# anatshafir1/bpp-phyl

Hardware: AMD Instinct MI355X
Metric: site-pattern x node partial updates/s (higher is better)
Workload: dtype f64

## Files before the change

bpp-phyl_amd/csrc/plk.hip:

```cpp

#include "../../include/plk.h"
#include "plk_kernels.hpp"
#include "plk_tree4.hpp"
#include "plk_deriv.hpp"
#include "plk_mfma64.hpp"
#include "plk_treeM.hpp"
#include "plk_jit.hpp"
#include "plk_jitm.hpp"
#include "plk_dr.hpp"
#include "plk_post.hpp"
#include "plk_map.hpp"
#include "plk_nni.hpp"
#include "plk_rell.hpp"
#include "plk_pair.hpp"
#include "plk_pars.hpp"
#include "plk_sim.hpp"
#include "plk_smap.hpp"
#include "plk_exchange.hpp"

#include <hip/hip_runtime.h>
#include <hip/hiprtc.h>
#include <rccl/rccl.h>

#include <sys/stat.h>
// ... 280 lines not shown
  double* d_cls = nullptr;
  size_t d_cls_cap = 0;
  double* fused_cls_blocks = nullptr;
  bool cls_site_written = false;
  uint8_t* d_ucodes_dc = nullptr;
  size_t ucodes_dc_cap = 0;
  bool ucodes_dc_valid = false;
  int ucodes_dc_w = 0;
  int32_t* d_units_start = nullptr;
  size_t units_start_cap = 0;
  uint8_t* d_ucodes = nullptr;
  int4* d_units = nullptr;
  size_t ucodes_cap = 0, units_cap = 0;
  bool ucodes_valid = false;
  int jit_resident = 0;
  std::string kernel_path;
  std::vector<std::vector<uint8_t> > tip_codes_host;
  bool cmp_valid = false;
  bool slots_expanded = false;
  std::vector<plk_op> cmp_ops;
  std::vector<std::vector<int32_t> > cmp_ids;
  std::vector<int64_t> cmp_D;
  std::vector<int> cmp_level_start, cmp_level_maxD;
  uint32_t* d_links = nullptr;
  size_t d_links_cap = 0;
  KOpL* d_opsl = nullptr;
  KKid* d_kidsl = nullptr;
  size_t d_kidsl_cap = 0;
  size_t d_opsl_cap = 0;
  int64_t cmp_work = 0;
// ... 226 lines not shown
int collect_events(plk_handle h) {
  if (h->events.empty()) return PLK_OK;
  HIPCHK(h, hipStreamSynchronize(h->stream));
  for (auto& e : h->events) {
    float ms = 0.f;
    HIPCHK(h, hipEventElapsedTime(&ms, e.a, e.b));
    h->acc_ms[e.kind] += ms;
    h->event_pool.push_back(e);
  }
  h->events.clear();
  return PLK_OK;
}

std::mutex g_jit_mutex;
std::map<std::pair<int, std::string>, hipFunction_t> g_jit_cache;
std::map<std::string, std::vector<char> > g_jit_code;

std::string jit_cache_dir() {
  const char* e = env_get("PLK_JIT_CACHE");
  if (e && (e[0] == '0' || e[0] == '\0')) return std::string();
  std::string d;
  if (e) {
    d = e;
  } else if (const char* x = env_get("XDG_CACHE_HOME")) {
    d = std::string(x) + "/plk_jit";
  } else if (const char* hm = env_get("HOME")) {
    d = std::string(hm) + "/.cache/plk_jit";
  } else {
    return std::string();
  }
// ... 85 lines not shown
  hiprtcDestroyProgram(&prog);
  if (log)
    std::fprintf(stderr, "[plk] jit compiled %zu bytes of source in %.2f s\n", src.size(),
                 std::chrono::duration<double>(std::chrono::steady_clock::now() - t0).count());
  if (!stem.empty()) {
    write_file_atomic(stem + ".co", code->data(), code->size());
    const std::string sm = code_sum(*code);
    write_file_atomic(stem + ".sum", sm.data(), sm.size());
    write_file_atomic(stem + ".hip", src.data(), src.size());
  }
  return PLK_OK;
}

int jit_function(plk_handle h, const std::string& src, const char* name, hipFunction_t* out) {
  std::lock_guard<std::mutex> lock(g_jit_mutex);
  const auto key = std::make_pair(h->device, src);
  auto it = g_jit_cache.find(key);
  if (it != g_jit_cache.end()) {
    *out = it->second;
    return PLK_OK;
  }
  auto ct = g_jit_code.find(src);
  bool from_cache = false;
  if (ct == g_jit_code.end()) {
    std::vector<char> code;
    if (int rc = jit_compile(h, src, &code, false, &from_cache)) return rc;
    ct = g_jit_code.emplace(src, std::move(code)).first;
  }
  std::vector<char>& code = ct->second;
  if (const char* dir = env_get("PLK_JIT_DUMP")) {
    const std::string stem = std::string(dir) + "/plk_jit_" + std::to_string(g_jit_cache.size());
    if (FILE* f = std::fopen((stem + ".hip").c_str(), "wb")) {
      std::fwrite(src.data(), 1, src.size(), f);
      std::fclose(f);
// ... 6 lines not shown
  hipSetDevice(h->device);
  hipModule_t mod;
  auto load = [&]() {
    try {
      return hipModuleLoadData(&mod, code.data()) == hipSuccess;
    } catch (...) {
      return false;
    }
  };
  if (!load()) {
    if (!from_cache) return fail(h, PLK_ERR_DEVICE, "hipModuleLoadData of the compiled tree kernel failed");
    (void)hipGetLastError();
    if (int rc = jit_compile(h, src, &code, true, &from_cache)) return rc;
    if (!load()) return fail(h, PLK_ERR_DEVICE, "hipModuleLoadData of the recompiled tree kernel failed");
  }
  hipFunction_t fn;
  HIPCHK(h, hipModuleGetFunction(&fn, mod, name));
  g_jit_cache.emplace(key, fn);
  *out = fn;
  return PLK_OK;
}

bool s4_supported(int C) { return C == 1 || C == 2 || C == 4 || C == 8; }

constexpr int kDerivScratch = 6;
constexpr int kScratchMats = 4;
constexpr int kScratchTips = 4;

template <bool SCALE>
void launch_s4(plk_handle h, const KOp* d_ops, int n_ops, const PartialsArgs& a) {
// ... 79 lines not shown
    return PLK_OK;
  if (!h->table_set) return fail(h, PLK_ERR_STATE, "code table not set (plk_set_code_table)");
  for (int t = 0; t < h->n_tips; ++t)
    if (!h->pmat_valid[t]) return fail(h, PLK_ERR_STATE, "transition matrix of tip branch %d not set", t);
  if (h->n_tips > 0) {
    dim3 grid(h->n_tips, h->C);
    if (h->S == 64)
      tip_table64_kernel<<<grid, 256, (size_t)(64 * 64 + h->n_codes * 64) * sizeof(double), h->stream>>>(
          h->pmats, h->code_table, h->tipP, h->n_tips, h->C, h->n_codes);
    else
      tip_table_kernel<<<grid, 256, 0, h->stream>>>(h->pmats, h->code_table, h->tipP, h->n_tips, h->C, h->S,
                                                    h->n_codes);
    HIPCHK(h, hipGetLastError());
  }
  std::fill(h->tip_table_valid.begin(), h->tip_table_valid.end(), 1);
  return PLK_OK;
}

int upload_compact_table(plk_handle h) {
  const int S = h->S;
  const int U = std::max((int)h->code_orig.size(), 1);
  std::vector<double> t((size_t)U * S, 0.0);
  for (size_t k = 0; k < h->code_orig.size(); ++k)
    std::copy(h->code_table_host.begin() + (size_t)h->code_orig[k] * S,
              h->code_table_host.begin() + (size_t)(h->code_orig[k] + 1) * S, t.begin() + k * S);
  hipSetDevice(h->device);
  HIPCHK(h, hipStreamSynchronize(h->stream));
  HIPCHK(h, hipMemcpy(h->code_table, t.data(), t.size() * sizeof(double), hipMemcpyHostToDevice));
  h->n_codes = U;
  h->tip_table_valid.assign(h->n_tips, 0);
  return PLK_OK;
}

int multi_forward(plk_handle h, int rc) {
  if (rc) {
    h->last_error = std::string("shard: ") + g_last_error;
    for (plk_handle s : h->shards)
      if (!s->last_error.empty()) h->last_error = "shard: " + s->last_error;
  }
  return rc;
}

int multi_run(plk_handle h, const std::function<int(size_t)>& f) {
  const size_t n = h->shards.size();
  if (n == 1) {
// ... 15 lines not shown

int multi_slices(plk_handle h, const std::function<int(plk_handle, int64_t)>& f) {
  return multi_run(h, [&](size_t i) { return f(h->shards[i], h->shard_start[i]); });
}

}

extern "C" {
int root_launch_c(plk_handle h, int root, double* site_lnl);
int root_finish_c(plk_handle h, double* lnl, double* block_sums);
}

namespace {
double* block_target(plk_handle h);
int launch_cls_blocks(plk_handle h, int guard, int32_t* uflow, bool site);

int32_t* uflow_arm(plk_handle h) {
  if (h->flags & PLK_FLAG_SCALING) return nullptr;
  *(volatile int32_t*)h->h_uflow = 0;
  return h->d_uflow;
}

size_t shard_block0(plk_handle h, size_t i) { return (size_t)(h->shard_start[i] / kRootBlock); }

void sum_blocks(const std::vector<double>& all, double* lnl, double* block_sums) {
  double s = 0.0;
  for (double v : all) s += v;
  if (lnl) *lnl = s;
  if (block_sums) std::memcpy(block_sums, all.data(), all.size() * sizeof(double));
}
// ... 226 lines not shown
    delete h;
    return PLK_OK;
  }
  hipSetDevice(h->device);
  if (h->stream) hipStreamSynchronize(h->stream);
  comm_release(h);
  void* bufs[] = {h->partials, h->scale, h->codes, h->code_table, h->tipP, h->pmats, h->dpmats, h->d2pmats,
                  h->V, h->Vinv, h->lambda, h->weights, h->rates, h->probs, h->pi, h->site_lnl,
                  h->d_ops, h->wave_sums, h->d_links, h->d_opsl, h->d_prog, h->d_frag, h->d1_sums,
                  h->d2_sums, h->d_dprog, h->pmatsT, h->d_ucodes, h->d_units, h->d_cherry3,
                  h->d_cherry_tips, h->d_cherry, h->d_drb, h->d_drm, h->dr_blk, h->dr_out, h->d_drpre, h->d_sbctr,
                  h->d_cherry_rows, h->d_kidsl, h->d_cls, h->d_ucodes_dc, h->d_units_start, h->d_post, h->post_buf,
                  h->count_G, h->wmats, h->d_mapb, h->map_blk, h->d_mapreq, h->d_nni, h->nni_vit, h->d_pair,
                  h->rell_rows, h->rell_W, h->rell_stage, h->rell_bad, h->pars_sets, h->pars_scores, h->d_pars,
                  h->d_pars_moves, h->sim_states, h->d_sim, h->d_smap_tab, h->d_smap_pois, h->d_smap_list,
                  h->d_smap_sums, h->d_smap_work, h->d_smap_keep};
  for (void* p : bufs)
    if (p) hipFree(p);
  if (h->h_req) (void)hipHostFree(h->h_req);
  if (h->h_blocks) hipHostFree(h->h_blocks);
  if (h->h_uflow) hipHostFree(h->h_uflow);
  if (h->h_clk) hipHostFree(h->h_clk);
  if (h->h_nni) (void)hipHostFree(h->h_nni);
  if (h->req_done) hipEventDestroy(h->req_done);
  for (auto& e : h->events) {
    hipEventDestroy(e.a);
    hipEventDestroy(e.b);
  }
  for (auto& e : h->event_pool) {
    hipEventDestroy(e.a);
    hipEventDestroy(e.b);
// ... 293 lines not shown
  a.mask = deriv_mask;
  a.n_req = n;
  a.uni_model = -1;
  if (h->S == 64) {
    a.uni_model = model ? model[0] : 0;
    for (int i = 1; model && i < n; ++i)
      if (model[i] != a.uni_model) a.uni_model = -1;
  }
  const bool k64 = h->S == 64 && deriv_mask == PLK_DERIV_P;
  const bool tips_fused = h->table_set && (h->S <= 20 || (k64 && h->n_codes <= 64));
  a.init = tips_fused ? h->code_table : nullptr;
  a.tipP = h->tipP;
  a.n_tips = h->n_tips;
  a.n_codes = h->n_codes;
  TimedSpan span(h, PLK_TIME_PMAT, 1);
  const size_t lds = (size_t)(h->S + (tips_fused ? 3 : 2) * S2) * sizeof(double);
  const bool pk_generic = !k64 && h->S != 4;
  if ((k64 || pk_generic) && (deriv_mask & PLK_DERIV_P)) a.PT = h->pmatsT;
  if (k64) {
    const int rx = tune_int("P64RX", 4, 0, 4), nb = tune_int("P64NB", 2, 1, 4);
    if (rx == 0) {
      pmat64s_kernel<<<dim3(n, h->C, 4), dim3(256), (size_t)(64 + 16 * 64 + S2) * sizeof(double), h->stream>>>(a, inl);
    } else {
      const int rr = rx <= 1 ? 1 : rx <= 2 ? 2 : 4, nn = nb <= 1 ? 1 : nb <= 2 ? 2 : 4;
      const dim3 g((unsigned)((n * h->C + nn - 1) / nn), (unsigned)(64 / (4 * rr)));
      const size_t lds = (size_t)(64 * kP64Pad + nn * 64 + nn * 4 * rr * kP64Pad) * sizeof(double);
#define PLK_P64W(RX_, NB_) \
  if (rr == RX_ && nn == NB_) pmat64w_kernel<RX_, NB_><<<g, dim3(256), lds, h->stream>>>(a, inl);
      PLK_P64W(1, 1) PLK_P64W(1, 2) PLK_P64W(1, 4) PLK_P64W(2, 1) PLK_P64W(2, 2) PLK_P64W(2, 4)
      PLK_P64W(4, 1) PLK_P64W(4, 2) PLK_P64W(4, 4)
#undef PLK_P64W
    }
  } else if (h->S == 4)
  {
    const dim3 g4((unsigned)((n * h->C * 4 + 63) / 64));
    if (inl.n > 0 && inl.n <= kPmatInlineSmall) {
      PmatInlineSmall sm;
      sm.n = inl.n;
      std::copy(inl.t, inl.t + inl.n, sm.t);
      std::copy(inl.branch, inl.branch + inl.n, sm.branch);
      std::copy(inl.model, inl.model + inl.n, sm.model);
      pmat4_kernel<PmatInlineSmall><<<g4, dim3(64), 0, h->stream>>>(a, sm);
    } else {
      pmat4_kernel<PmatInline><<<g4, dim3(64), 0, h->stream>>>(a, inl);
    }
  }
  else
// ... 8 lines not shown
  }
  HIPCHK(h, hipGetLastError());
  if (inl.n == 0) {
    if (h->in_eval)
      h->req_unrecorded = true;
    else
      HIPCHK(h, hipEventRecord(h->req_done, h->stream));
  }
  span.stop();
  if (deriv_mask & PLK_DERIV_P) {
    for (int i = 0; i < n; ++i) {
      h->pmat_valid[branch[i]] = 1;
      if (!a.PT) h->pmatsT_dirty = true;
      if (branch[i] < h->n_tips) h->tip_table_valid[branch[i]] = tips_fused ? 1 : 0;
    }
  }
  if (h->deriv_valid.empty()) h->deriv_valid.assign(h->n_nodes, 0);
  const bool both = (deriv_mask & (PLK_DERIV_P | PLK_DERIV_DP | PLK_DERIV_D2P)) ==
                    (PLK_DERIV_P | PLK_DERIV_DP | PLK_DERIV_D2P);
  for (int i = 0; i < n; ++i) h->deriv_valid[branch[i]] = both ? 1 : 0;
  return PLK_OK;
}

int plk_set_pmatrix(plk_handle h, int branch, const double* P) {
  env_refresh();
  if (h && !h->shards.empty()) return multi_each(h, [&](plk_handle x) { return plk_set_pmatrix(x, branch, P); });
  if (!h || !P || branch < 0 || branch >= h->n_nodes) return fail(h, PLK_ERR_ARG, "bad branch %d", branch);
  hipSetDevice(h->device);
  HIPCHK(h, hipStreamSynchronize(h->stream));
  const size_t n = (size_t)h->C * h->S * h->S;
  HIPCHK(h, hipMemcpy(h->pmats + (size_t)branch * n, P, n * sizeof(double), hipMemcpyHostToDevice));
  h->pmat_valid[branch] = 1;
  h->state_epoch++;
  h->pmatsT_dirty = true;
  if (!h->deriv_valid.empty()) h->deriv_valid[branch] = 0;
  if (branch < h->n_tips) h->tip_table_valid[branch] = 0;
  return PLK_OK;
}

int plk_get_dpmatrix(plk_handle h, int branch, int order, double* dP) {
  env_refresh();
  if (h && !h->shards.empty()) return multi_forward(h, plk_get_dpmatrix(h->shards[0], branch, order, dP));
  if (!h || !dP || branch < 0 || branch >= h->n_nodes || (order != 1 && order != 2))
    return fail(h, PLK_ERR_ARG, "bad derivative request (branch %d, order %d)", branch, order);
  const double* src = order == 1 ? h->dpmats : h->d2pmats;
  if (!src) return fail(h, PLK_ERR_STATE, "no derivative matrices (PLK_DERIV_DP / PLK_DERIV_D2P)");
  hipSetDevice(h->device);
  HIPCHK(h, hipStreamSynchronize(h->stream));
  const size_t n = (size_t)h->C * h->S * h->S;
  HIPCHK(h, hipMemcpy(dP, src + (size_t)branch * n, n * sizeof(double), hipMemcpyDeviceToHost));
  return PLK_OK;
// ... 298 lines not shown
  for (int i = 0; i < nf; ++i) {
    start_sorted[i] = start[order[i]];
    start_sorted[nf + i] = res_first[order[i]];
    if (h->prog_tiers.empty() || tier[order[i]] != tier[order[i - 1]]) h->prog_tiers.push_back({});
    h->prog_tiers.back().push_back(i);
  }
  HIPCHK(h, hipMemcpyAsync(h->d_frag, start_sorted.data(), 2 * nf * sizeof(int32_t), hipMemcpyHostToDevice,
                           h->stream));
  h->prog_nf = nf;
  rc = ensure_cap(h, (void**)&h->d_sbctr, &h->d_sbctr_cap, (size_t)(nf * h->C + 1) * sizeof(unsigned));
  if (rc) return rc;
  HIPCHK(h, hipMemsetAsync(h->d_sbctr, 0, (size_t)(nf * h->C + 1) * sizeof(unsigned), h->stream));
  h->prog_host = prog;
  h->frag_starts_host.assign(start_sorted.begin(), start_sorted.begin() + nf);
  h->jit_fn = nullptr;
  h->jitm_fn = nullptr;
  h->jit_plan_valid = false;
  HIPCHK(h, hipStreamSynchronize(h->stream));
  h->prog_ops.assign(ops, ops + n_ops);
  h->prog_materialize = materialize;
  h->prog_reduce = reduce;
  h->prog_dm = DM;
  h->prog_jit = jit_tree4(h);
  h->prog_jitm = jit_treeM(h);
  h->prog_ciw = jit_ciw(h);
  h->prog_tmax = TMAX;
  h->prog_root = root_reduce;
  h->cherry3.swap(cherry3);
  h->cherry_codes_valid = false;
  h->prog_mat_after.assign(h->n_internal, -1);
// ... 134 lines not shown
  const bool cls_ok = !h->prog_ciw && !scale && (h->flags & PLK_FLAG_LNL_ONLY) && U <= 4;
  const int qb = cls_ok ? tune_int("JIT_QUAD_KB", 136, 0, 150) * 1024 / (int)sizeof(double) : 0;
  if (h->jit_plan_valid && h->jit_plan_U == U && h->jit_plan_budget == budget && h->jit_plan_qb == qb) return;
  h->jit_plan_cls = false;
  if (qb > 0) {
    h->jit_plan = jit_plan(h->prog_host, h->frag_starts_host, h->C, U, std::max(qb, budget), scale, true, qb);
    for (const auto& un : h->jit_plan.units)
      for (const JitUnit& u : un) h->jit_plan_cls |= u.tc >= 0;
  }
  if (!h->jit_plan_cls) h->jit_plan = jit_plan(h->prog_host, h->frag_starts_host, h->C, U, budget, scale);
  h->jit_plan_valid = true;
  h->jit_plan_U = U;
  h->jit_plan_budget = budget;
  h->jit_plan_qb = qb;
  h->jit_fn = nullptr;
  h->ucodes_valid = false;
}

int jit4_shape(plk_handle h, JitShape& sh) {
  sh.C = h->C;
  sh.CW = h->prog_ciw ? h->C : 1;
  sh.pin = true;
  sh.U = h->n_codes;
  sh.scale = (h->flags & PLK_FLAG_SCALING) != 0;
  jit4_ensure_plan(h, sh.U, sh.scale);
  sh.cls = h->jit_plan_cls;
  sh.NT = h->jit_plan.NU;
  sh.TD = h->jit_plan.tab_doubles;
  sh.QT = h->jit_plan.quad_tmp;
  sh.soa = tune_int("JIT_SOA", 1, 0, 1) != 0;
// ... 2 lines not shown
  sh.dcw = sh.NT <= 16 ? 1 : 2;
  sh.ps1 = tune_int("JIT_PS1", 0, 0, 1) != 0;
  sh.PW = tune_int("JIT_PW", sh.dc && sh.cls ? 2 : 1, 1, 2);
  sh.G = tune_int("JIT_G", 0, 0, 16);
  if (sh.G == 0) {
    if (sh.cls) {
      sh.G = 16;
      while (sh.G > 1 && sh.lds_bytes() > 160 * 1024 - 64) --sh.G;
    } else {
      sh.G = h->prog_ciw ? 8 : sh.scale ? 1 : jit_auto_groups(sh);
    }
  }
  sh.G = std::max(1, std::min(sh.G, 1024 / (64 * sh.nw())));
  sh.wt = sh.wt_ok() && tune_int("JIT_WT", sh.cls ? 1 : 0, 0, 1) != 0;
  sh.wp = sh.wt && tune_int("JIT_WP", sh.cls ? 1 : 0, 0, 1) != 0;
  sh.L = tune_int("JIT_L", h->prog_ciw ? 2 : 3, 1, 8);
  sh.RD = tune_int("JIT_RD", 1, 1, 8);
  sh.minw = 0;
  sh.ppipe = true;
  sh.clk = env_is("PLK_DEBUG_CLOCK", '1') ? 1 : env_is("PLK_DEBUG_CLOCK", '2') ? 2 : env_is("PLK_DEBUG_CLOCK", '3') ? 3 : 0;
  if (sh.lds_bytes() > 160 * 1024 - 64)
    return fail(h, PLK_ERR_UNSUPPORTED, "tree kernel needs %zu B of LDS", sh.lds_bytes());
  return PLK_OK;
}

int jit4_unit_codes(plk_handle h, const JitShape& sh) {
  if (!h->ucodes_valid) {
    std::vector<int4> units;
    for (const auto& un : h->jit_plan.units)
      for (const JitUnit& u : un) units.push_back(make_int4(u.ta, u.tb, u.tc, u.td));
// ... 22 lines not shown
    HIPCHK(h, hipMemcpyAsync(h->d_units_start, us.data(), us.size() * sizeof(int32_t), hipMemcpyHostToDevice,
                             h->stream));
    const dim3 dg((unsigned)((h->n_pad + 255) / 256), (unsigned)nfr);
    hipLaunchKernelGGL(unit_codes_dc_kernel, dg, dim3(256), 0, h->stream, h->d_ucodes, h->n_pad, h->d_units_start,
                       sh.dcw, reinterpret_cast<uint4*>(h->d_ucodes_dc));
    HIPCHK(h, hipGetLastError());
    HIPCHK(h, hipStreamSynchronize(h->stream));
    h->ucodes_dc_valid = true;
    h->ucodes_dc_w = sh.dcw;
  }
  return PLK_OK;
}

int jit4_compile(plk_handle h, const JitShape& sh) {
  if (h->jit_fn && sh == h->jit_shape) return PLK_OK;
  int rc = jit_function(h, jit_tree4_source(h->jit_plan, sh), jit_tree4_name(sh), &h->jit_fn);
  if (rc) return rc;
  h->jit_shape = sh;
  h->jit_resident = 0;
  return PLK_OK;
}

int jit4_args(plk_handle h, int32_t* uflow, JArgs& ja) {
  const JitShape& sh = h->jit_shape;
  fill_common_args(h, uflow, ja);
  ja.codes = sh.dc ? h->d_ucodes_dc : h->d_ucodes;
  ja.tipP = h->tipP;
  ja.n_sblocks = (int32_t)((h->n_pad + 64 * sh.G * sh.PW - 1) / (64 * sh.G * sh.PW));
  ja.n_tasks = (int32_t)((h->n_pad + 64 * sh.PW - 1) / (64 * sh.PW));
  ja.sb_ctr = h->d_sbctr;
  ja.cls_sum = nullptr;
  if (sh.cls) {
    int rc = ensure_cap(h, (void**)&h->d_cls, &h->d_cls_cap, (size_t)h->C * h->n_pad * sizeof(double));
    if (rc) return rc;
    ja.cls_sum = h->d_cls;
  }
  return PLK_OK;
}

int jitm_compile(plk_handle h) {
  JitMShape msh;
  msh.S = h->S;
  msh.C = h->C;
  msh.U = h->n_codes;
  msh.scale = (h->flags & PLK_FLAG_SCALING) != 0;
  msh.L = tune_int("JITM_L", 1, 1, 4);
  msh.minw = 2;
  msh.pd = 1;
  msh.pipe = 2;
  msh.lc = 3;
  msh.G = 4;
// ... 103 lines not shown
  }
  TreeArgs a;
  const size_t lds = tree_args(h, a);
  size_t lds_m = 0;
  if (kind == FK_TREEM) {
    if (int rc = treeM_staging(h, a, lds_m)) return rc;
  }
  const bool jit = h->prog_jit;
  JArgs ja;
  if (jit) {
    JitShape sh;
    int rc = jit4_shape(h, sh);
    if (!rc) rc = jit4_unit_codes(h, sh);
    if (!rc) rc = jit4_compile(h, sh);
    if (!rc) rc = jit4_args(h, a.uflow, ja);
    if (rc) return rc;
  }
  const bool jitm = kind == FK_TREEM && h->prog_jitm;
  JMArgs ma;
  if (jitm) {
    if (int rc = jitm_compile(h)) return rc;
    jitm_args(h, a.uflow, ma);
  }
  h->kernel_path = jit ? "jit_tree4" : jitm ? "jit_treeM" : kind == FK_TREEM ? "treeM" : "tree4";
  h->fused_cls_blocks = nullptr;
  if (jit && h->jit_shape.clk) {
    if (int rc = grow_clock_stamps(h)) return rc;
  }
  int first = 0;
  for (const auto& t : h->prog_tiers) {
// ... 4039 lines not shown
```

bpp-phyl_amd/csrc/plk_jit.hpp:

```cpp
#pragma once

#include <algorithm>
#include <string>
#include <tuple>
#include <vector>

#include "plk_tree4.hpp"

namespace plk {

static const char* kJitPrelude = R"PLKJIT(
typedef unsigned char u8;
typedef long long i64;
typedef int i32;
typedef __attribute__((address_space(4))) const double* CPd;
#define kTile 128
#define kLn2x256 177.44567822334599921
#define kScaleUp 115792089237316195423570985008687907853269984665640564039457584007913129639936.0
#define kScaleThr (1.0 / kScaleUp)

struct JArgs {  // codes: one row per table unit (unit_codes_kernel)
  double* partials; i32* scale; const u8* codes; const double* tipP; const double* weights;
  const double* pi; const double* probs; double* site_lnl; double* wave_sums;
  i64 slot_stride; i64 n_pad; i64 n_patterns; i32 n_sblocks; i32 guard;
// ... 353 lines not shown
  const double* pi;
  const double* probs;
  double* site_lnl;
  double* wave_sums;
  int64_t slot_stride;
  int64_t n_pad;
  int64_t n_patterns;
  int32_t n_sblocks;
  int32_t guard;
  unsigned* sb_ctr;
  int32_t dyn;
  unsigned* exit_ctr;
  int32_t* uflow;
  double* cls_sum;
  int32_t n_tasks;
};
static const char* kJitArgsTail = "[C][n_pad]\n};";
static const char* kJitArgsTailWt = "[C][n_pad]\n  i32 n_tasks;  // wave tasks (64 * PW_ patterns each)\n};";

struct JitShape {
  int C = 1;
  int CW = 1;
  int PW = 1;
  bool pin = false;
  int G = 1;
  int U = 1;
  int NT = 0;
  int TD = 0;
  bool scale = false;
  int L = 1;
  int RD = 1;
  int minw = 0;
  bool ppipe = true;
  int clk = 0;
  bool cls = false;
  int QT = 0;
  bool soa = false;
  bool ps1 = false;
  bool dc = false;
  int dcw = 1;
  bool wt = false;
  bool wp = false;
  auto tied() const {
    return std::tie(C, CW, PW, pin, G, U, NT, TD, scale, L, RD, minw, ppipe, clk, cls, QT, soa, ps1, dc, dcw, wt, wp);
  }
  bool operator==(const JitShape& o) const { return tied() == o.tied(); }
  int nw() const { return cls ? 1 : C / CW; }
  bool wt_ok() const { return dc && nw() == 1; }
  size_t lds_bytes() const {
    const size_t nt = (size_t)std::max(NT, 1);
    const size_t xch = cls ? 0 : (scale ? 2 : 1) * (size_t)PW * G * nw() * 64 * sizeof(double);
    return (size_t)std::max(TD, 4) * sizeof(double) + xch +
           std::max(dc ? (size_t)0 : (size_t)G * nt * 64 * PW, (size_t)QT * sizeof(double));
  }
};

#define PLK_POOL_TASK_EXPR(x, gx, j) ((x) + (j) * (gx))
#define PLK_STR_(...) #__VA_ARGS__
#define PLK_STR(...) PLK_STR_(__VA_ARGS__)
inline int jit_pool_task(int x, int gx, int j) { return PLK_POOL_TASK_EXPR(x, gx, j); }

inline const char* jit_tree4_name(const JitShape& sh) { return sh.cls ? "plk_jit_tree4c" : "plk_jit_tree4"; }

inline int jit_auto_groups(const JitShape& base) {
  int best_g = 1, best_w = 0;
  for (int g = 1; g <= 4; ++g) {
    JitShape t = base;
    t.G = g;
    const int waves_wg = t.nw() * g;
    const int by_lds = (int)((160 * 1024) / std::max<size_t>(t.lds_bytes(), 1));
    const int by_vgpr = (4 * 7) / waves_wg;
    const int waves = std::min(by_lds, by_vgpr) * waves_wg;
    if (waves > best_w) {
      best_w = waves;
      best_g = g;
    }
  }
// ... 104 lines not shown
      off += u.tb < 0 ? single : u.tc >= 0 ? quad : pair;
      if (u.koff >= 0) {
        u.koff = off;
        off += (U * U + 31) / 32 * 4;
      }
    }
    plan.NU = std::max(plan.NU, (int)un.size());
    plan.tab_doubles = std::max(plan.tab_doubles, off);
    int nq = 0;
    for (const JitUnit& u : un) nq += u.tc >= 0;
    plan.quad_tmp = std::max(plan.quad_tmp, 2 * nq * U * U * 4);
  }
  return plan;
}

inline std::string jit_tree4_source(const JitPlan& plan, const JitShape& sh) {
  const std::vector<std::vector<JitEvent> >& events = plan.events;
  const int C = sh.C, L = std::max(sh.L, 1), U = sh.U;
  std::string s;
  s.reserve(4096 * events.size() + 16384);
  s += sh.ppipe ? "#define PPIPE_ 1\n" : "#define PPIPE_ 0\n";
  s += kJitPrelude;
  if (sh.wt) {
    const size_t at = s.find(kJitArgsTail);
    if (at == std::string::npos) return std::string();
    s.replace(at, std::string(kJitArgsTail).size(), kJitArgsTailWt);
  }
  char buf[400];
  const std::string minw_s = sh.minw > 0 ? ", " + std::to_string(sh.minw) : std::string();
  std::string ud = "};\nstruct __attribute__((aligned(32))) UnitD { int ta, tb, off, br, koff, p0, p1, p2; };\n"
                   "__device__ const UnitD kUnitD[] = {{0, 0, 0, 0, 0, 0, 0, 0}";
  std::string sc = "};\n__device__ const int kFragScStart[] = {0", scu = "};\n__device__ const int kScUnit[] = {0",
              ot = "};\n__device__ const int kFragOtherStart[] = {0",
              otu = "};\n__device__ const UnitD kOtherD[] = {{0, 0, 0, 0, 0, 0, 0, 0}";
  std::string qs = "};\nstruct QuadD { int ta, tb, tc, td, brA, brB, brQ, off; };\n"
                   "__device__ const int kFragQuadStart[] = {0",
              qd = "};\n__device__ const QuadD kQuadD[] = {{0, 0, 0, 0, 0, 0, 0, 0}";
  {
    std::string st = "\n__device__ const int kFragPStart[] = {0", br = "};\n__device__ const int kFragPBr[] = {0";
    int acc = 0;
    for (size_t f = 0; f < events.size(); ++f) {
// ... 150 lines not shown
  // (issued before the table staging below: its loads overlap it)
  if (DC_) fetch_dc(blockIdx.x); else fetch_codes(blockIdx.x);
)PLKJIT";
  else
    s += R"PLKJIT(  auto fetch_dc = [&](int tk_) {
    const i64 q0_ = (i64)tk_ * (64 * PW_);
    const i64 pp_ = (q0_ < a.n_pad ? q0_ : 0) + lane;
    if (tk_ < a.n_tasks)
      _Pragma("unroll") for (int pw = 0; pw < PW_; ++pw)
        _Pragma("unroll") for (int w_ = 0; w_ < DCW_; ++w_) cvn_[pw][w_] = dcodes[(pp_ + 64 * pw) * DCW_ + w_];
  };
  (void)cv_; (void)cvn_; (void)dcodes; (void)fetch_codes;
  // (issued before the table staging below: its loads overlap it)
  fetch_dc((int)blockIdx.x * G_ + g);
)PLKJIT";
  s += R"PLKJIT(  // The fragment's P(t) matrices, touched with wide loads while the tables stage: the
  // traversal reads P(t) through scalar loads one contribution ahead, and their first touch
  // (with one class per wave (cfg2) the first super-block shows no such penalty and the
  // touch only lengthened the staging, so there it is left out)
  double ptouch_ = 0.0;
  if (CW_ > 1) {
    const int pb0 = 1 + kFragPStart[frag], npb = kFragPStart[frag + 1] - kFragPStart[frag];
    const double2* pp_ = reinterpret_cast<const double2*>(pmats);
    for (int i = threadIdx.x; i < npb * C_ * 8; i += 64 * NWT_) {
      const int k_ = i / (C_ * 8);
      ptouch_ += pp_[(i64)kFragPBr[pb0 + k_] * (C_ * 8) + (i - k_ * (C_ * 8))].x;
    }
  }
  if (SC_) {
    // rescaling contribution units: one (unit, row) per thread; each row all classes, the
    // cherry's joint check as rescale() makes it, then contrib<.., true>
// ... 136 lines not shown
      __builtin_amdgcn_wave_barrier();
      __builtin_amdgcn_fence(__ATOMIC_ACQUIRE, "wavefront");
      _Pragma("unroll") for (int r = lane; r < U4_; r += 64) {
        const int ab = r / (U_ * U_), cd = r - ab * (U_ * U_);
        const double2* pa = reinterpret_cast<const double2*>(qtmp + ((i64)(2 * kk) * (U_ * U_) + ab) * 4);
        const double2* pb = reinterpret_cast<const double2*>(qtmp + ((i64)(2 * kk + 1) * (U_ * U_) + cd) * 4);
        const double2 a0 = pa[0], a1 = pa[1], b0 = pb[0], b1 = pb[1];
        double acc[4] = {a0.x, a0.y, a1.x, a1.y}, o[4];
        acc[0] *= b0.x; acc[1] *= b0.y; acc[2] *= b1.x; acc[3] *= b1.y;
        pcon(PQ, acc, o);
        *reinterpret_cast<double2*>(tab + qd_.off + TABIX(U4_, QROW_(r), 0)) = make_double2(o[0], o[1]);
        *reinterpret_cast<double2*>(tab + qd_.off + TABIX(U4_, QROW_(r), 2)) = make_double2(o[2], o[3]);
      }
    }
  }
  const CPd pm = (CPd)(pmats + c0 * 16);
  const double* trow = tab + (CLS_ ? 0 : c0 * (U_ * 4));         // single-tip units
  const double* trow2 = tab + (CLS_ ? 0 : c0 * (U_ * U_ * 4));   // pair units
  const double* trow4 = tab;                                      // quad units (CLS_ only)
  (void)xch; (void)xch2; (void)trow; (void)trow2; (void)trow4;
// unit k: codes of the lane's patterns (4 per int), then their table rows (R rows per
// class at OFF doubles from the class base TB)
#define CODEF(Q, k) { Q = 0; _Pragma("unroll") for (int pw_ = 0; pw_ < PW_; ++pw_) \
    Q |= (DC_ ? (int)((cvw(cv_[pw_][(k) >> 4], ((k) >> 2) & 3) >> (8 * ((k) & 3))) & 255) : (int)crow[(k) * (64 * PW_) + 64 * pw_]) << (8 * pw_); }
#define ROWF(F, TB, OFF, R, Q) { _Pragma("unroll") for (int pw_ = 0; pw_ < PW_; ++pw_) { \
    const double* r0_ = TB + (OFF) + TABIX(R, ((Q) >> (8 * pw_)) & 255, 0); \
    _Pragma("unroll") for (int cw_ = 0; cw_ < CW_; ++cw_) { \
      const double2* r_ = reinterpret_cast<const double2*>(r0_ + cw_ * ((R) * 4)); \
      const double2 x_ = r_[0], y_ = r_[SOA_ ? (R) : 1]; const int v_ = 4 * (pw_ * CW_ + cw_); \
      F[v_] = x_.x; F[v_ + 1] = x_.y; F[v_ + 2] = y_.x; F[v_ + 3] = y_.y; } } }
#define TIPF(F, Q, k, TB, OFF, R) { CODEF(Q, k) ROWF(F, TB, OFF, R, Q) }
// ... 342 lines not shown
    s += "  if (threadIdx.x == 0) {\n"
         "    unsigned long long* q_ = clk_ + 4 * (((unsigned long long)blockIdx.z * gridDim.y + blockIdx.y) * gridDim.x + "
         "blockIdx.x);\n"
         "    const unsigned long long c1_ = clock64(), w1_ = wall_clock64();\n"
         "    q_[0] = clk_c0_; q_[1] = clk_w0_; q_[2] = c1_; q_[3] = w1_;\n  }\n";
  s += R"PLKJIT(  if (a.exit_ctr && threadIdx.x == 0) {
    const unsigned t_ = __hip_atomic_fetch_add(a.exit_ctr, 1u, __ATOMIC_RELAXED, __HIP_MEMORY_SCOPE_AGENT);
    if (t_ == gridDim.x * gridDim.y * gridDim.z - 1u) {
      for (unsigned f_ = 0; f_ < gridDim.y * gridDim.z; ++f_)
        __hip_atomic_store(a.sb_ctr + frag_base * gridDim.z + f_, 0u, __ATOMIC_RELAXED, __HIP_MEMORY_SCOPE_AGENT);
      __hip_atomic_store(a.exit_ctr, 0u, __ATOMIC_RELAXED, __HIP_MEMORY_SCOPE_AGENT);
    }
  }
}
)PLKJIT";
  if (sh.clk == 2) {
    const std::string anchor = sh.wt ? "  for (int tk_nx = 0; tk < a.n_tasks; tk = tk_nx) {"
                                     : "  for (int sb = blockIdx.x, sb_nx = 0; sb < a.n_sblocks; sb = sb_nx) {";
    const size_t at = s.find(anchor);
    if (at != std::string::npos)
      s.insert(at, "  if (threadIdx.x == 0) { unsigned long long* q_ = clk_ + 4 * (((unsigned long long)blockIdx.z * "
                   "gridDim.y + blockIdx.y) * gridDim.x + blockIdx.x); const unsigned long long c1_ = clock64(), w1_ = "
                   "wall_clock64(); q_[0] = clk_c0_; q_[1] = clk_w0_; q_[2] = c1_; q_[3] = w1_; }\n");
  }
  if (sh.clk == 3) {
    const std::string head = sh.wt ? "  for (int tk_nx = 0; tk < a.n_tasks; tk = tk_nx) {"
                                   : "  for (int sb = blockIdx.x, sb_nx = 0; sb < a.n_sblocks; sb = sb_nx) {";
    const std::string bar = "    __syncthreads();  // (DC_: also the tables' staging before the first super-block)\n";
    const std::string tail = "    default: break;\n    }\n  }\n";
    size_t at = s.rfind(tail);
// ... 30 lines not shown
```

Measured before the change: 772.3 billion.

## Precompute per-fragment tip/pair/quad table images in the P(t) kernel

Adds a JIT-compiled table-image kernel that builds each fragment's per-class tip, pair and quad lookup tables in global memory, fused with the P(t) computation when branch lengths change. The tree kernel then copies these ready-made images into shared memory instead of building the tables per block during staging, which removes redundant per-block table construction and the P(t) touch. The cost is an extra image buffer, added invalidation bookkeeping, and a launch that must be kept consistent with the pmat and tip-table state. The JIT cache is also rekeyed by function name so one module can expose several kernels.

```diff
diff --git a/bpp-phyl_amd/csrc/plk.hip b/bpp-phyl_amd/csrc/plk.hip
--- a/bpp-phyl_amd/csrc/plk.hip
+++ b/bpp-phyl_amd/csrc/plk.hip
@@ -318,6 +318,12 @@
   size_t ucodes_cap = 0, units_cap = 0;
   bool ucodes_valid = false;
   int jit_resident = 0;
+  double* d_tab_img = nullptr;
+  size_t tab_img_cap = 0;
+  bool tab_img_valid = false;
+  hipFunction_t jit_tabs_fn[2] = {nullptr, nullptr};
+  int tab_units = 0;
+  std::vector<int> tab_branches;
   std::string kernel_path;
   std::vector<std::vector<uint8_t> > tip_codes_host;
   bool cmp_valid = false;
@@ -574,6 +580,7 @@
 
 std::mutex g_jit_mutex;
 std::map<std::pair<int, std::string>, hipFunction_t> g_jit_cache;
+std::map<std::pair<int, std::string>, hipModule_t> g_jit_modules;
 std::map<std::string, std::vector<char> > g_jit_code;
 
 std::string jit_cache_dir() {
@@ -689,10 +696,18 @@
 
 int jit_function(plk_handle h, const std::string& src, const char* name, hipFunction_t* out) {
   std::lock_guard<std::mutex> lock(g_jit_mutex);
-  const auto key = std::make_pair(h->device, src);
+  const auto key = std::make_pair(h->device, std::string(name) + "\n" + src);
   auto it = g_jit_cache.find(key);
   if (it != g_jit_cache.end()) {
     *out = it->second;
+    return PLK_OK;
+  }
+  auto mt = g_jit_modules.find(std::make_pair(h->device, src));
+  if (mt != g_jit_modules.end()) {
+    hipFunction_t fn;
+    HIPCHK(h, hipModuleGetFunction(&fn, mt->second, name));
+    g_jit_cache.emplace(key, fn);
+    *out = fn;
     return PLK_OK;
   }
   auto ct = g_jit_code.find(src);
@@ -729,6 +744,7 @@
     if (int rc = jit_compile(h, src, &code, true, &from_cache)) return rc;
     if (!load()) return fail(h, PLK_ERR_DEVICE, "hipModuleLoadData of the recompiled tree kernel failed");
   }
+  g_jit_modules.emplace(std::make_pair(h->device, src), mod);
   hipFunction_t fn;
   HIPCHK(h, hipModuleGetFunction(&fn, mod, name));
   g_jit_cache.emplace(key, fn);
@@ -838,6 +854,7 @@
     HIPCHK(h, hipGetLastError());
   }
   std::fill(h->tip_table_valid.begin(), h->tip_table_valid.end(), 1);
+  h->tab_img_valid = false;
   return PLK_OK;
 }
 
@@ -853,6 +870,7 @@
   HIPCHK(h, hipMemcpy(h->code_table, t.data(), t.size() * sizeof(double), hipMemcpyHostToDevice));
   h->n_codes = U;
   h->tip_table_valid.assign(h->n_tips, 0);
+  h->tab_img_valid = false;
   return PLK_OK;
 }
 
@@ -898,6 +916,8 @@
 namespace {
 double* block_target(plk_handle h);
 int launch_cls_blocks(plk_handle h, int guard, int32_t* uflow, bool site);
+bool tab_image_serves(plk_handle h, unsigned deriv_mask, bool tips_fused);
+int launch_tab_image(plk_handle h, const PmatArgs& a, const PmatInline& inl);
 
 int32_t* uflow_arm(plk_handle h) {
   if (h->flags & PLK_FLAG_SCALING) return nullptr;
@@ -1154,7 +1174,7 @@
                   h->count_G, h->wmats, h->d_mapb, h->map_blk, h->d_mapreq, h->d_nni, h->nni_vit, h->d_pair,
                   h->rell_rows, h->rell_W, h->rell_stage, h->rell_bad, h->pars_sets, h->pars_scores, h->d_pars,
                   h->d_pars_moves, h->sim_states, h->d_sim, h->d_smap_tab, h->d_smap_pois, h->d_smap_list,
-                  h->d_smap_sums, h->d_smap_work, h->d_smap_keep};
+                  h->d_smap_sums, h->d_smap_work, h->d_smap_keep, h->d_tab_img};
   for (void* p : bufs)
     if (p) hipFree(p);
   if (h->h_req) (void)hipHostFree(h->h_req);
@@ -1478,6 +1498,7 @@
   a.n_tips = h->n_tips;
   a.n_codes = h->n_codes;
   TimedSpan span(h, PLK_TIME_PMAT, 1);
+  bool built_image = false;
   const size_t lds = (size_t)(h->S + (tips_fused ? 3 : 2) * S2) * sizeof(double);
   const bool pk_generic = !k64 && h->S != 4;
   if ((k64 || pk_generic) && (deriv_mask & PLK_DERIV_P)) a.PT = h->pmatsT;
@@ -1495,6 +1516,9 @@
       PLK_P64W(4, 1) PLK_P64W(4, 2) PLK_P64W(4, 4)
 #undef PLK_P64W
     }
+  } else if (h->S == 4 && tab_image_serves(h, deriv_mask, tips_fused)) {
+    built_image = true;
+    if (int rc = launch_tab_image(h, a, inl)) return rc;
   } else if (h->S == 4)
   {
     const dim3 g4((unsigned)((n * h->C * 4 + 63) / 64));
@@ -1533,6 +1557,12 @@
       if (!a.PT) h->pmatsT_dirty = true;
       if (branch[i] < h->n_tips) h->tip_table_valid[branch[i]] = tips_fused ? 1 : 0;
     }
+  }
+  h->tab_img_valid = false;
+  if (built_image) {
+    h->tab_img_valid = true;
+    for (int b : h->tab_branches)
+      if (!h->pmat_valid[b] || (b < h->n_tips && !h->tip_table_valid[b])) h->tab_img_valid = false;
   }
   if (h->deriv_valid.empty()) h->deriv_valid.assign(h->n_nodes, 0);
   const bool both = (deriv_mask & (PLK_DERIV_P | PLK_DERIV_DP | PLK_DERIV_D2P)) ==
@@ -1554,6 +1584,7 @@
   h->pmatsT_dirty = true;
   if (!h->deriv_valid.empty()) h->deriv_valid[branch] = 0;
   if (branch < h->n_tips) h->tip_table_valid[branch] = 0;
+  h->tab_img_valid = false;
   return PLK_OK;
 }
 
@@ -1882,6 +1913,7 @@
   h->prog_host = prog;
   h->frag_starts_host.assign(start_sorted.begin(), start_sorted.begin() + nf);
   h->jit_fn = nullptr;
+  h->tab_img_valid = false;
   h->jitm_fn = nullptr;
   h->jit_plan_valid = false;
   HIPCHK(h, hipStreamSynchronize(h->stream));
@@ -2046,6 +2078,7 @@
   h->jit_plan_budget = budget;
   h->jit_plan_qb = qb;
   h->jit_fn = nullptr;
+  h->tab_img_valid = false;
   h->ucodes_valid = false;
 }
 
@@ -2078,6 +2111,7 @@
   sh.G = std::max(1, std::min(sh.G, 1024 / (64 * sh.nw())));
   sh.wt = sh.wt_ok() && tune_int("JIT_WT", sh.cls ? 1 : 0, 0, 1) != 0;
   sh.wp = sh.wt && tune_int("JIT_WP", sh.cls ? 1 : 0, 0, 1) != 0;
+  sh.img = sh.cls && tune_int("JIT_IMG", 1, 0, 1) != 0;
   sh.L = tune_int("JIT_L", h->prog_ciw ? 2 : 3, 1, 8);
   sh.RD = tune_int("JIT_RD", 1, 1, 8);
   sh.minw = 0;
@@ -2130,10 +2164,88 @@
 
 int jit4_compile(plk_handle h, const JitShape& sh) {
   if (h->jit_fn && sh == h->jit_shape) return PLK_OK;
-  int rc = jit_function(h, jit_tree4_source(h->jit_plan, sh), jit_tree4_name(sh), &h->jit_fn);
+  h->tab_img_valid = false;
+  h->jit_tabs_fn[0] = h->jit_tabs_fn[1] = nullptr;
+  const std::string src = jit_tree4_source(h->jit_plan, sh);
+  int rc = jit_function(h, src, jit_tree4_name(sh), &h->jit_fn);
   if (rc) return rc;
+  if (sh.img) {
+    for (int l = 0; l < 2 && !rc; ++l) rc = jit_function(h, src, jit_tabs4_name(l != 0), &h->jit_tabs_fn[l]);
+    const size_t bytes = h->jit_plan.units.size() * (size_t)h->C * std::max(sh.TD, 4) * sizeof(double);
+    const size_t cap0 = h->tab_img_cap;
+    if (!rc) rc = ensure_cap(h, (void**)&h->d_tab_img, &h->tab_img_cap, bytes);
+    if (!rc && h->tab_img_cap != cap0) HIPCHK(h, hipMemsetAsync(h->d_tab_img, 0, h->tab_img_cap, h->stream));
+    if (rc) {
+      h->jit_fn = nullptr;
+      return rc;
+    }
+    h->tab_units = 0;
+    h->tab_branches.clear();
+    for (const auto& un : h->jit_plan.units)
+      for (const JitUnit& u : un) {
+        ++h->tab_units;
+        for (int b : {u.ta, u.tb, u.tc, u.td, u.br, u.brA, u.brB})
+          if (b >= 0) h->tab_branches.push_back(b);
+      }
+  }
   h->jit_shape = sh;
   h->jit_resident = 0;
+  return PLK_OK;
+}
+
+bool tab_image_serves(plk_handle h, unsigned deriv_mask, bool tips_fused) {
+  return h->S == 4 && deriv_mask == PLK_DERIV_P && tips_fused && h->jit_fn && h->jit_plan_valid && h->jit_plan_cls &&
+         h->jit_shape.img && h->jit_shape.U == h->n_codes && h->jit_tabs_fn[0] && h->jit_tabs_fn[1] && h->d_tab_img &&
+         !tune_is("JIT_IMG", '0');
+}
+
+int launch_tab_image(plk_handle h, const PmatArgs& a, const PmatInline& inl) {
+  PmatArgs pa = a;
+  double* img = h->d_tab_img;
+  int nlead = (pa.n_req * h->C * 4 + 255) / 256;
+  const unsigned grid = (unsigned)(nlead + h->tab_units * h->C);
+  if (grid == 0) return PLK_OK;
+  if (inl.n <= kPmatInlineSmall) {
+    PmatInlineSmall sm;
+    sm.n = inl.n;
+    std::copy(inl.t, inl.t + inl.n, sm.t);
+    std::copy(inl.branch, inl.branch + inl.n, sm.branch);
+    std::copy(inl.model, inl.model + inl.n, sm.model);
+    void* args[] = {&pa, &sm, &img, &nlead};
+    HIPCHK(h, hipModuleLaunchKernel(h->jit_tabs_fn[0], grid, 1, 1, 256, 1, 1, 0, h->stream, args, nullptr));
+  } else {
+    PmatInline full = inl;
+    void* args[] = {&pa, &full, &img, &nlead};
+    HIPCHK(h, hipModuleLaunchKernel(h->jit_tabs_fn[1], grid, 1, 1, 256, 1, 1, 0, h->stream, args, nullptr));
+  }
+  return PLK_OK;
+}
+
+int jit4_table_image(plk_handle h) {
+  if (!h->jit_shape.img || h->tab_img_valid) return PLK_OK;
+  for (int b : h->tab_branches)
+    if (!h->pmat_valid[b]) return fail(h, PLK_ERR_STATE, "transition matrix of branch %d not set", b);
+  PmatArgs a;
+  std::memset(&a, 0, sizeof(a));
+  a.rates = h->rates;
+  a.V = h->V;
+  a.Vinv = h->Vinv;
+  a.lambda = h->lambda;
+  a.P = h->pmats;
+  a.init = h->code_table;
+  a.tipP = h->tipP;
+  a.n_tips = h->n_tips;
+  a.n_codes = h->n_codes;
+  a.S = h->S;
+  a.C = h->C;
+  a.mask = PLK_DERIV_P;
+  a.uni_model = -1;
+  PmatInline inl;
+  inl.n = 0;
+  TimedSpan span(h, PLK_TIME_TABLES, 3);
+  if (int rc = launch_tab_image(h, a, inl)) return rc;
+  if (span.stop()) h->n_table_launches++;
+  h->tab_img_valid = true;
   return PLK_OK;
 }
 
@@ -2151,6 +2263,7 @@
     if (rc) return rc;
     ja.cls_sum = h->d_cls;
   }
+  ja.tab_img = h->d_tab_img;
   return PLK_OK;
 }
 
@@ -2284,6 +2397,7 @@
     if (!rc) rc = jit4_unit_codes(h, sh);
     if (!rc) rc = jit4_compile(h, sh);
     if (!rc) rc = jit4_args(h, a.uflow, ja);
+    if (!rc) rc = jit4_table_image(h);
     if (rc) return rc;
   }
   const bool jitm = kind == FK_TREEM && h->prog_jitm;
diff --git a/bpp-phyl_amd/csrc/plk_jit.hpp b/bpp-phyl_amd/csrc/plk_jit.hpp
--- a/bpp-phyl_amd/csrc/plk_jit.hpp
+++ b/bpp-phyl_amd/csrc/plk_jit.hpp
@@ -391,9 +391,13 @@
   int32_t* uflow;
   double* cls_sum;
   int32_t n_tasks;
+  const double* tab_img;
 };
 static const char* kJitArgsTail = "[C][n_pad]\n};";
 static const char* kJitArgsTailWt = "[C][n_pad]\n  i32 n_tasks;  // wave tasks (64 * PW_ patterns each)\n};";
+static const char* kJitArgsTailImg =
+    "[C][n_pad]\n  i32 n_tasks;  // wave tasks (64 * PW_ patterns each)\n"
+    "  const double* tab_img;  // table images [fragment][class][TD_], in the layout of tab\n};";
 
 struct JitShape {
   int C = 1;
@@ -418,8 +422,10 @@
   int dcw = 1;
   bool wt = false;
   bool wp = false;
+  bool img = false;
   auto tied() const {
-    return std::tie(C, CW, PW, pin, G, U, NT, TD, scale, L, RD, minw, ppipe, clk, cls, QT, soa, ps1, dc, dcw, wt, wp);
+    return std::tie(C, CW, PW, pin, G, U, NT, TD, scale, L, RD, minw, ppipe, clk, cls, QT, soa, ps1, dc, dcw, wt, wp,
+                    img);
   }
   bool operator==(const JitShape& o) const { return tied() == o.tied(); }
   int nw() const { return cls ? 1 : C / CW; }
@@ -428,7 +434,7 @@
     const size_t nt = (size_t)std::max(NT, 1);
     const size_t xch = cls ? 0 : (scale ? 2 : 1) * (size_t)PW * G * nw() * 64 * sizeof(double);
     return (size_t)std::max(TD, 4) * sizeof(double) + xch +
-           std::max(dc ? (size_t)0 : (size_t)G * nt * 64 * PW, (size_t)QT * sizeof(double));
+           std::max(dc ? (size_t)0 : (size_t)G * nt * 64 * PW, img ? (size_t)0 : (size_t)QT * sizeof(double));
   }
 };
 
@@ -438,6 +444,7 @@
 inline int jit_pool_task(int x, int gx, int j) { return PLK_POOL_TASK_EXPR(x, gx, j); }
 
 inline const char* jit_tree4_name(const JitShape& sh) { return sh.cls ? "plk_jit_tree4c" : "plk_jit_tree4"; }
+inline const char* jit_tabs4_name(bool large) { return large ? "plk_jit_tabs4c_l" : "plk_jit_tabs4c"; }
 
 inline int jit_auto_groups(const JitShape& base) {
   int best_g = 1, best_w = 0;
@@ -572,6 +579,245 @@
   return plan;
 }
 
+static const char* kJitImgCopy = R"PLKJIT(  double ptouch_ = 0.0;
+  {
+    const double2* src_ = reinterpret_cast<const double2*>(a.tab_img + ((i64)frag * C_ + c0) * TD_);
+    double2* dst_ = reinterpret_cast<double2*>(tab);
+    constexpr int NV_ = 8, NH_ = TD_ / 2, RS_ = NV_ * 64 * NWT_;
+    _Pragma("nounroll") for (int k0_ = 0; k0_ < NH_; k0_ += RS_) {
+      double2 r_[NV_];
+      _Pragma("unroll") for (int q_ = 0; q_ < NV_; ++q_) {
+        const int k_ = k0_ + (int)threadIdx.x + 64 * NWT_ * q_;
+        r_[q_] = src_[k_ < NH_ ? k_ : 0];
+      }
+      _Pragma("unroll") for (int q_ = 0; q_ < NV_; ++q_) {
+        const int k_ = k0_ + (int)threadIdx.x + 64 * NWT_ * q_;
+        if (k_ < NH_) dst_[k_] = r_[q_];
+      }
+    }
+  }
+)PLKJIT";
+
+inline std::string jit_tabs4_source(const JitPlan& plan) {
+  std::string qf = "__device__ const int kQuadFrag[] = {0", of = "};\n__device__ const int kOtherFrag[] = {0";
+  char buf[64];
+  int nq = 0, no = 0;
+  for (size_t f = 0; f < plan.units.size(); ++f)
+    for (const JitUnit& u : plan.units[f]) {
+      snprintf(buf, sizeof(buf), ",%zu", f);
+      if (u.tc >= 0) {
+        qf += buf;
+        ++nq;
+      } else {
+        of += buf;
+        ++no;
+      }
+    }
+  std::string s = qf + of + "};\n";
+  snprintf(buf, sizeof(buf), "#define NQA_ %d\n#define NOA_ %d\n", nq, no);
+  s += buf;
+  s += R"PLKJIT(struct PmatArgs {  // (plk_kernels.hpp: the same fields in the same order)
+  const i32* branch; const i32* model; const double* t; const double* rates; const double* V; const double* Vinv;
+  const double* lambda; double* P; double* PT; double* dP; double* d2P; const double* init; double* tipP;
+  int n_tips, n_codes; int S, C; unsigned mask; int n_req; int uni_model;
+};
+template <int N> struct PmatInl { double t[N]; i32 branch[N]; i32 model[N]; i32 n; };
+// row x of P(t) for class c of a request entry (length t, model m)
+__device__ __forceinline__ void pmat4_row(const PmatArgs& a, double t, int m, int c, int x, double (&p)[4]) {
+  constexpr int S = 4;
+  const double rc = a.rates[c];
+  const double tt = t * rc;
+  const double* V = a.V + (size_t)m * S * S;
+  const double* Vi = a.Vinv + (size_t)m * S * S;
+  const double* lam = a.lambda + (size_t)m * S;
+  double e[S], l[S], vx[S], vi[S * S];
+#pragma unroll
+  for (int k = 0; k < S; ++k) {
+    l[k] = lam[k];
+    vx[k] = V[x * S + k];
+  }
+#pragma unroll
+  for (int k = 0; k < S * S; ++k) vi[k] = Vi[k];
+#pragma unroll
+  for (int k = 0; k < S; ++k) e[k] = exp(l[k] * tt);
+#pragma unroll
+  for (int y = 0; y < S; ++y) {
+    p[y] = 0.0;
+#pragma unroll
+    for (int k = 0; k < S; ++k) {
+      const double w = vx[k] * vi[k * S + y];
+      p[y] = __builtin_fma(w, e[k], p[y]);
+    }
+    if (tt == 0.0) p[y] = (x == y) ? 1.0 : 0.0;  // getPij_t: t == 0 -> identity
+  }
+}
+// entry x of a tip's table row of one code: sum_y P[x][y] init[code][y]
+__device__ __forceinline__ double tip4_entry(const PmatArgs& a, const double (&p)[4], int code) {
+  double t = 0.0;
+#pragma unroll
+  for (int y = 0; y < 4; ++y) t = __builtin_fma(p[y], a.init[code * 4 + y], t);
+  return t;
+}
+template <class Inl>
+__device__ __forceinline__ void tabs4_body(const PmatArgs& a, const Inl& inl, double* __restrict__ img, int nlead) {
+  const int tid = threadIdx.x;
+  if ((int)blockIdx.x < nlead) {
+    const int gid = blockIdx.x * 256 + tid;
+    if (gid >= a.n_req * C_ * 4) return;
+    const int x = gid & 3, ic = gid >> 2, i = ic / C_, c = ic - i * C_;
+    const int b = inl.n ? inl.branch[i] : a.branch[i];
+    const int m = inl.n ? inl.model[i] : (a.model ? a.model[i] : 0);
+    double p[4];
+    pmat4_row(a, inl.n ? inl.t[i] : a.t[i], m, c, x, p);
+    const size_t off = ((size_t)b * C_ + c) * 16 + x * 4;
+#pragma unroll
+    for (int y = 0; y < 4; ++y) a.P[off + y] = p[y];
+    if (a.init && b < a.n_tips) {
+      double* out = a.tipP + ((size_t)b * C_ + c) * (U_ * 4) + x;
+      for (int code = 0; code < U_; ++code) out[code * 4] = tip4_entry(a, p, code);
+    }
+    return;
+  }
+  __shared__ __attribute__((aligned(16))) double sT_[4][U_ * 4];  // the unit's tips' table rows of this class
+  __shared__ __attribute__((aligned(16))) double sP_[3][16];      // P(t) of its branches (cherry, or A, B, Q)
+  __shared__ __attribute__((aligned(16))) double sQ_[2 * U_ * U_ * 4];  // a quad's two cherries' contribution rows
+  __shared__ int sIdx_[8];                                        // request entry of tips 0..3, branches 0..2 (-1: none)
+  const int ub = (int)blockIdx.x - nlead, k = ub / C_, c0 = ub - k * C_;
+  int tp[4], br[3], off, frag;
+  if (k < NQA_) {
+    const QuadD q = kQuadD[1 + k];
+    tp[0] = q.ta; tp[1] = q.tb; tp[2] = q.tc; tp[3] = q.td;
+    br[0] = q.brA; br[1] = q.brB; br[2] = q.brQ;
+    off = q.off;
+    frag = kQuadFrag[1 + k];
+  } else {
+    const UnitD u = kOtherD[1 + k - NQA_];
+    tp[0] = u.ta; tp[1] = u.tb; tp[2] = -1; tp[3] = -1;
+    br[0] = u.br; br[1] = -1; br[2] = -1;
+    off = u.off;
+    frag = kOtherFrag[1 + k - NQA_];
+  }
+  double* dst = img + ((i64)frag * C_ + c0) * TD_ + off;
+  if (tid < 8) sIdx_[tid] = -1;
+  __syncthreads();
+  for (int i = tid; i < a.n_req; i += 256) {
+    const int b = inl.n ? inl.branch[i] : a.branch[i];
+#pragma unroll
+    for (int j = 0; j < 4; ++j)
+      if (b == tp[j]) sIdx_[j] = i;
+#pragma unroll
+    for (int j = 0; j < 3; ++j)
+      if (b == br[j]) sIdx_[4 + j] = i;
+  }
+  __syncthreads();
+  if (tid < 4 * U_ * 4) {  // tip j, row q = code * 4 + x
+    const int j = tid / (U_ * 4), q = tid - j * (U_ * 4);
+    const int tip = j == 0 ? tp[0] : j == 1 ? tp[1] : j == 2 ? tp[2] : tp[3];
+    if (tip >= 0) {
+      const int i = sIdx_[j];
+      double v;
+      if (i >= 0) {
+        double p[4];
+        pmat4_row(a, inl.n ? inl.t[i] : a.t[i], inl.n ? inl.model[i] : (a.model ? a.model[i] : 0), c0, q & 3, p);
+        v = tip4_entry(a, p, q >> 2);
+      } else {
+        v = a.tipP[((i64)tip * C_ + c0) * (U_ * 4) + q];
+      }
+      sT_[j][q] = v;
+    }
+  } else if (tid >= 64 && tid < 64 + 48) {  // branch j, element e = x * 4 + y
+    const int j = (tid - 64) >> 4, e = (tid - 64) & 15;
+    const int b = j == 0 ? br[0] : j == 1 ? br[1] : br[2];
+    if (b >= 0) {
+      const int i = sIdx_[4 + j];
+      double v;
+      if (i >= 0) {
+        double p[4];
+        pmat4_row(a, inl.n ? inl.t[i] : a.t[i], inl.n ? inl.model[i] : (a.model ? a.model[i] : 0), c0, e >> 2, p);
+        const int y = e & 3;
+        v = y == 0 ? p[0] : y == 1 ? p[1] : y == 2 ? p[2] : p[3];
+      } else {
+        v = a.P[((i64)b * C_ + c0) * 16 + e];
+      }
+      sP_[j][e] = v;
+    }
+  }
+  __syncthreads();
+  auto pcon = [&](const double* P, const double (&v_)[4], double (&t_)[4]) {
+    _Pragma("unroll") for (int x = 0; x < 4; ++x) {
+      t_[x] = P[4 * x] * v_[0];
+      t_[x] = __builtin_fma(P[4 * x + 1], v_[1], t_[x]);
+      t_[x] = __builtin_fma(P[4 * x + 2], v_[2], t_[x]);
+      t_[x] = __builtin_fma(P[4 * x + 3], v_[3], t_[x]);
+    }
+  };
+  if (tp[1] < 0) {  // a tip's rows
+    for (int i = tid; i < U_ * 4; i += 256) dst[TABIX(U_, i >> 2, i & 3)] = sT_[0][i];
+  } else if (tp[2] < 0) {
+    // a pair: one row (code pair ca, cb) per thread; through P of the cherry's branch where the
+    // unit holds the cherry's contribution (contrib<.., true>: the same operations in the same order)
+    for (int q = tid; q < U_ * U_; q += 256) {
+      const int ca = q / U_, cb = q - ca * U_;
+      const double2* pa = reinterpret_cast<const double2*>(&sT_[0][ca * 4]);
+      const double2* pb = reinterpret_cast<const double2*>(&sT_[1][cb * 4]);
+      const double2 a0 = pa[0], a1 = pa[1], b0 = pb[0], b1 = pb[1];
+      const double v[4] = {a0.x * b0.x, a0.y * b0.y, a1.x * b1.x, a1.y * b1.y};
+      double2* o0 = reinterpret_cast<double2*>(dst + TABIX(U_ * U_, q, 0));
+      double2* o1 = reinterpret_cast<double2*>(dst + TABIX(U_ * U_, q, 2));
+      if (br[0] < 0) {
+        *o0 = make_double2(v[0], v[1]);
+        *o1 = make_double2(v[2], v[3]);
+      } else {
+        double t[4];
+        pcon(sP_[0], v, t);
+        *o0 = make_double2(t[0], t[1]);
+        *o1 = make_double2(t[2], t[3]);
+      }
+    }
+  } else {
+    // a quad.  Phase 1: 2 U^2 threads form the two cherries' contribution rows; phase 2: one quad
+    // row per thread from them (the interpreter's order: each cherry's pair product and
+    // contrib<.., true> through the cherry's P, Q's accumulator = contA, *= contB, then
+    // contrib<.., true> through P_Q)
+    constexpr int U4_ = U_ * U_ * U_ * U_;
+    for (int hr = tid; hr < 2 * U_ * U_; hr += 256) {
+      const int which = hr / (U_ * U_), r = hr - which * (U_ * U_), ca = r / U_, cb = r - ca * U_;
+      const double2* pa = reinterpret_cast<const double2*>(&sT_[2 * which][ca * 4]);
+      const double2* pb = reinterpret_cast<const double2*>(&sT_[2 * which + 1][cb * 4]);
+      const double2 a0 = pa[0], a1 = pa[1], b0 = pb[0], b1 = pb[1];
+      const double v[4] = {a0.x * b0.x, a0.y * b0.y, a1.x * b1.x, a1.y * b1.y};
+      double o[4];
+      pcon(sP_[which], v, o);
+      double2* od = reinterpret_cast<double2*>(sQ_ + hr * 4);
+      od[0] = make_double2(o[0], o[1]);
+      od[1] = make_double2(o[2], o[3]);
+    }
+    __syncthreads();
+    for (int r = tid; r < U4_; r += 256) {
+      const int ab = r / (U_ * U_), cd = r - ab * (U_ * U_);
+      const double2* pa = reinterpret_cast<const double2*>(sQ_ + ab * 4);
+      const double2* pb = reinterpret_cast<const double2*>(sQ_ + (U_ * U_ + cd) * 4);
+      const double2 a0 = pa[0], a1 = pa[1], b0 = pb[0], b1 = pb[1];
+      double acc[4] = {a0.x, a0.y, a1.x, a1.y}, o[4];
+      acc[0] *= b0.x; acc[1] *= b0.y; acc[2] *= b1.x; acc[3] *= b1.y;
+      pcon(sP_[2], acc, o);
+      *reinterpret_cast<double2*>(dst + TABIX(U4_, QROW_(r), 0)) = make_double2(o[0], o[1]);
+      *reinterpret_cast<double2*>(dst + TABIX(U4_, QROW_(r), 2)) = make_double2(o[2], o[3]);
+    }
+  }
+}
+extern "C" __global__ __launch_bounds__(256) void plk_jit_tabs4c(PmatArgs a, const PmatInl<64> inl,
+                                                                 double* __restrict__ img, int nlead) {
+  tabs4_body(a, inl, img, nlead);
+}
+extern "C" __global__ __launch_bounds__(256) void plk_jit_tabs4c_l(PmatArgs a, const PmatInl<160> inl,
+                                                                   double* __restrict__ img, int nlead) {
+  tabs4_body(a, inl, img, nlead);
+}
+)PLKJIT";
+  return s;
+}
+
 inline std::string jit_tree4_source(const JitPlan& plan, const JitShape& sh) {
   const std::vector<std::vector<JitEvent> >& events = plan.events;
   const int C = sh.C, L = std::max(sh.L, 1), U = sh.U;
@@ -579,10 +825,11 @@
   s.reserve(4096 * events.size() + 16384);
   s += sh.ppipe ? "#define PPIPE_ 1\n" : "#define PPIPE_ 0\n";
   s += kJitPrelude;
-  if (sh.wt) {
+  if (sh.img && !sh.cls) return std::string();
+  if (sh.wt || sh.img) {
     const size_t at = s.find(kJitArgsTail);
     if (at == std::string::npos) return std::string();
-    s.replace(at, std::string(kJitArgsTail).size(), kJitArgsTailWt);
+    s.replace(at, std::string(kJitArgsTail).size(), sh.img ? kJitArgsTailImg : kJitArgsTailWt);
   }
   char buf[400];
   const std::string minw_s = sh.minw > 0 ? ", " + std::to_string(sh.minw) : std::string();
@@ -763,7 +1010,10 @@
   // (issued before the table staging below: its loads overlap it)
   fetch_dc((int)blockIdx.x * G_ + g);
 )PLKJIT";
-  s += R"PLKJIT(  // The fragment's P(t) matrices, touched with wide loads while the tables stage: the
+  if (sh.img)
+    s += kJitImgCopy;
+  else
+    s += R"PLKJIT(  // The fragment's P(t) matrices, touched with wide loads while the tables stage: the
   // traversal reads P(t) through scalar loads one contribution ahead, and their first touch
   // (with one class per wave (cfg2) the first super-block shows no such penalty and the
   // touch only lengthened the staging, so there it is left out)
@@ -930,7 +1180,8 @@
       }
     }
   }
-  const CPd pm = (CPd)(pmats + c0 * 16);
+)PLKJIT";
+  s += R"PLKJIT(  const CPd pm = (CPd)(pmats + c0 * 16);
   const double* trow = tab + (CLS_ ? 0 : c0 * (U_ * 4));         // single-tip units
   const double* trow2 = tab + (CLS_ ? 0 : c0 * (U_ * U_ * 4));   // pair units
   const double* trow4 = tab;                                      // quad units (CLS_ only)
@@ -1303,6 +1554,7 @@
   }
 }
 )PLKJIT";
+  if (sh.img) s += jit_tabs4_source(plan);
   if (sh.clk == 2) {
     const std::string anchor = sh.wt ? "  for (int tk_nx = 0; tk < a.n_tasks; tk = tk_nx) {"
                                      : "  for (int sb = blockIdx.x, sb_nx = 0; sb < a.n_sblocks; sb = sb_nx) {";
```

Result: faster. 791.1 billion, median of 6 (+2.4%).
